# MIT-SPARK/Hydra-GNN

Hardware: AMD Instinct MI355X
Metric: scene-graphs/sec (fwd+bwd) MP3D hetero batch (higher is better)
Workload: dtype f32

## Files before the change

### hydra-gnn_amd/csrc/gemm.hip

```cpp
#include <algorithm>

#include "gemm_tile.h"

namespace hmp {

KT_DEFINE(gemm)

template <int ROWS, int BK>
using TileSide = TileSlots<256, ROWS, BK>;
template <int ROWS, int BK>
using TileRegs = StageRegs<TileSide<ROWS, BK>::NV>;

template <int ROWS, int BK>
__device__ __forceinline__ void tile_load_edge(TileRegs<ROWS, BK>& t, const float* __restrict__ p, int ld, int kcontig, int r0,
                                               int R, int n_real, int aug, int k0, int kend, int vec) {
  using S = TileSide<ROWS, BK>;
#pragma unroll
  for (int i = 0; i < S::NV; ++i) {
    float4 val = make_float4(0.f, 0.f, 0.f, 0.f);
    if (kcontig) {
      int r, k4;
      S::slot_rk(i, r, k4);
      const int gr = r0 + r, gk = k0 + k4;
      if (gr < R && gk < kend) {
// ... 405 lines not shown
    P.M = g.M; P.N = g.N; P.K = g.K; P.lda = g.lda; P.ldb = g.ldb; P.ldc = g.ldc; P.n_real = g.n_real; P.aug_ones = g.aug_ones;
    P.nslices = cdiv(g.N, TT_NS);
    int ks = (int)(512.0 * ((double)g.K * P.nslices / work_total) / P.nslices + 0.5);
    if (ks > GEMM_TALL_SLABS) ks = GEMM_TALL_SLABS;
    if (ks < 1) ks = 1;
    P.kchunk = g.kchunk = cdiv(cdiv(g.K, ks), TT_BK) * TT_BK;
    P.ksplit = g.ksplit = cdiv(g.K, P.kchunk);
    P.block_start = start;
    start += P.ksplit * P.nslices;
  }
  static const int rc = [] {
    return hipFuncSetAttribute(reinterpret_cast<const void*>(&gemm_tn_tall_kernel), hipFuncAttributeMaxDynamicSharedMemorySize,
                               2 * TT_STAGE * (int)sizeof(float)) == hipSuccess ? 0 : 1;
  }();
  HMP_CHECK_ARG(rc == 0, "gemm: could not raise the dynamic LDS limit of the tall weight-gradient kernel");
  hipLaunchKernelGGL(gemm_tn_tall_kernel, dim3(start), dim3(256), 2 * TT_STAGE * sizeof(float), st, tb);
  HMP_LAUNCH_CHECK();
  return HMP_OK;
}

int gemm_launch(GemmBatch& gb, bool want_split, int max_slabs, hipStream_t st) {
  HMP_CHECK_ARG(gb.n >= 0 && gb.n <= GEMM_MAX_PROB, "gemm: %d problems", gb.n);
  if (gemm_x3_takes(gb, want_split)) return gemm_x3_launch(gb, want_split, max_slabs, st);
  if (want_split) {
    GemmPeel tall;
    gemm_peel(gb, tall_takes, tall);
    if (tall.n_taken > 0) {
      HMP_TRY(tall_launch(gb, tall, st));
      return gemm_launch_rest(gb, tall, [&](GemmBatch& rest) { return gemm_launch(rest, want_split, max_slabs, st); });
    }
  }
  int64_t tiles64 = 0;
  double work = 0.0;
  int max_k = 0;
  for (int i = 0; i < gb.n; ++i) {
    const GemmProblem& p = gb.p[i];
    HMP_CHECK_ARG(p.M >= 0 && p.N >= 0 && p.K >= 0, "gemm: negative size");
    tiles64 += (int64_t)cdiv(p.M, 64) * cdiv(p.N, 64);
    work += (double)p.M * p.N * p.K;
    max_k = p.K > max_k ? p.K : max_k;
  }
  if (tiles64 >= 1024 || work >= 1e9) {
    int64_t tiles128 = 0;
    for (int i = 0; i < gb.n; ++i) tiles128 += (int64_t)cdiv(gb.p[i].M, 128) * cdiv(gb.p[i].N, 128);
    const bool big_ok = env_switch("HMP_GEMM_BIG") != '0';
    int min_n = 1 << 30;
    for (int i = 0; i < gb.n; ++i) min_n = gb.p[i].N < min_n ? gb.p[i].N : min_n;
    if (big_ok && min_n >= 256 && work >= 1e9 && (tiles128 >= 256 || (want_split && max_k >= 8192)))
      return launch_cfg<2, 2, 32, 2, 2>(gb, want_split, max_slabs, st);
    return launch_cfg<2, 2, 32>(gb, want_split, max_slabs, st);
  }
  if (max_k <= 64) return launch_cfg<1, 1, 64>(gb, want_split, max_slabs, st);
  return launch_cfg<1, 1, 128>(gb, want_split, max_slabs, st);
}

}

extern "C" int hmp_gemm_f32(const float* d_a, int32_t lda, int32_t trans_a, const float* d_b, int32_t ldb, int32_t trans_b,
                            float* d_c, int32_t ldc, int32_t M, int32_t N, int32_t K, void* stream) {
  using namespace hmp;
  HMP_CHECK_ARG(d_a && d_b && d_c, "hmp_gemm_f32: null pointer");
  HMP_CHECK_ARG(M >= 0 && N >= 0 && K >= 0, "hmp_gemm_f32: negative size");
  HMP_CHECK_ARG(lda >= (trans_a ? M : K) && ldb >= (trans_b ? K : N) && ldc >= N, "hmp_gemm_f32: leading dimension too small");
  GemmBatch gb;
  memset(&gb, 0, sizeof(gb));
  gb.n = 1;
  GemmProblem& p = gb.p[0];
  p.A = d_a; p.B = d_b; p.C = d_c;
  p.M = M; p.N = N; p.K = K;
  p.lda = lda; p.ldb = ldb; p.ldc = ldc;
  p.trans_a = trans_a; p.trans_b = trans_b;
  p.n_real = N;
  p.epi = EPI_NONE;
  if (M == 0 || N == 0) return HMP_OK;
  return gemm_launch(gb, false, 1, (hipStream_t)stream);
}

extern "C" int hmp_gemm_grouped(const hmp_gemm_desc* d, int32_t n, int32_t route, int32_t want_split, int32_t max_slabs,
                                int32_t* ksplit_out, void* stream) {
  using namespace hmp;
  static const bool have_device = hmp_device_count() > 0;
  HMP_CHECK_ARG(have_device, "hmp_gemm_grouped: no gfx950 device visible");
  HMP_CHECK_ARG((d || n == 0) && n >= 0 && n <= GEMM_MAX_PROB, "hmp_gemm_grouped: %d problems (at most %d)", n, GEMM_MAX_PROB);
  HMP_CHECK_ARG(route >= 0 && route <= 2 && max_slabs >= 1, "hmp_gemm_grouped: route %d, max_slabs %d", route, max_slabs);
  for (int i = 0; i < n; ++i) {
    const hmp_gemm_desc& q = d[i];
    HMP_CHECK_ARG(q.A && q.B && q.C, "hmp_gemm_grouped: null pointer (problem %d)", i);
    HMP_CHECK_ARG(q.M >= 0 && q.N >= 0 && q.K >= 0, "hmp_gemm_grouped: negative size (problem %d)", i);
    HMP_CHECK_ARG(q.n_real == q.N - (q.aug_ones ? 1 : 0) && q.n_real >= 0, "hmp_gemm_grouped: n_real %d, N %d, aug_ones %d (problem %d)",
                  q.n_real, q.N, q.aug_ones, i);
    HMP_CHECK_ARG(q.lda >= (q.trans_a ? q.M : q.K) && q.ldb >= (q.trans_b ? q.K : q.n_real) && q.ldc >= q.N,
                  "hmp_gemm_grouped: leading dimension too small (problem %d)", i);
    HMP_CHECK_ARG(q.epi == EPI_NONE || (q.epi == EPI_ACTMASK && q.H && q.ldh >= q.N), "hmp_gemm_grouped: epilogue (problem %d)", i);
    HMP_CHECK_ARG(!q.Cadd || q.ldadd >= q.N, "hmp_gemm_grouped: ldadd too small (problem %d)", i);
    HMP_CHECK_ARG(q.drop_p >= 0.f && q.drop_p < 1.f, "hmp_gemm_grouped: drop_p %g (problem %d)", (double)q.drop_p, i);
    HMP_CHECK_ARG(!want_split || q.M == 0 || q.slab_stride >= (int64_t)q.M * q.ldc, "hmp_gemm_grouped: slab_stride (problem %d)", i);
    HMP_CHECK_ARG(route == 1 || !(q.a_bf16 || q.b_bf16 || q.c_bf16 || q.h_bf16), "hmp_gemm_grouped: bf16 operands on route %d", route);
    HMP_CHECK_ARG(route != 2 || (q.trans_a && !q.trans_b && q.epi == EPI_NONE && !q.Cadd),
                  "hmp_gemm_grouped: the direct kernel takes the plain TN form only (problem %d)", i);
  }
  hipStream_t st = (hipStream_t)stream;
  if (route == 2) {
    TnBatch tb;
    memset(&tb, 0, sizeof(tb));
    tb.n = n;
    for (int i = 0; i < n; ++i) {
      const hmp_gemm_desc& q = d[i];
      TnProblem& P = tb.p[i];
      P.A = (const float*)q.A; P.B = (const float*)q.B; P.C = (float*)q.C; P.slab_stride = q.slab_stride;
      P.M = q.M; P.N = q.N; P.K = q.K; P.lda = q.lda; P.ldb = q.ldb; P.ldc = q.ldc;
      P.n_real = q.n_real; P.aug_ones = q.aug_ones;
    }
    int ok = 0;
    HMP_TRY(gemm_tn_direct_launch(tb, max_slabs, &ok, st));
    if (ksplit_out)
      for (int i = 0; i < n; ++i) ksplit_out[i] = ok ? tb.p[i].ksplit : 0;
    return HMP_OK;
  }
  GemmBatch gb;
  memset(&gb, 0, sizeof(gb));
  gb.n = n;
  for (int i = 0; i < n; ++i) {
    const hmp_gemm_desc& q = d[i];
    GemmProblem& p = gb.p[i];
    p.A = (const float*)q.A; p.B = (const float*)q.B; p.C = (float*)q.C; p.H = (const float*)q.H;
    p.a_bf16 = q.a_bf16; p.b_bf16 = q.b_bf16; p.c_bf16 = q.c_bf16; p.h_bf16 = q.h_bf16;
    p.slab_stride = q.slab_stride;
    p.M = q.M; p.N = q.N; p.K = q.K;
    p.lda = q.lda; p.ldb = q.ldb; p.ldc = q.ldc; p.ldh = q.ldh;
    p.trans_a = q.trans_a; p.trans_b = q.trans_b;
    p.n_real = q.n_real; p.aug_ones = q.aug_ones;
    p.epi = q.epi; p.act = q.act;
    p.drop_on = q.drop_p > 0.f ? 1 : 0;
    p.drop.thresh = drop_thresh(q.drop_p); p.drop.scale = 1.f / (1.f - q.drop_p);
    p.Cadd = q.Cadd; p.ldadd = q.ldadd;
  }
  const int rc = route == 0 ? gemm_launch(gb, want_split != 0, max_slabs, st) : gemm_bf16_launch(gb, want_split != 0, max_slabs, st);
  if (ksplit_out)
    for (int i = 0; i < n; ++i) ksplit_out[i] = gb.p[i].ksplit;
  return rc;
}
```

### hydra-gnn_amd/csrc/gemm_direct.hip

```cpp
#include "device_fns.h"

namespace hmp {

KT_DEFINE(gemmd)

typedef float f32x16 __attribute__((ext_vector_type(16)));

__device__ __forceinline__ void reduce4(f32x16& acc, float* red , int w, int lane, float (&out)[4]) {
#pragma unroll
  for (int i = 0; i < 16; ++i) red[(w * 16 + i) * 64 + lane] = acc[i];
  __syncthreads();
#pragma unroll
  for (int j = 0; j < 4; ++j) {
    const int i = 4 * w + j;
    out[j] = (red[(0 * 16 + i) * 64 + lane] + red[(1 * 16 + i) * 64 + lane]) + (red[(2 * 16 + i) * 64 + lane] + red[(3 * 16 + i) * 64 + lane]);
  }
}

constexpr int TN_MAXI = 24;

__global__ __launch_bounds__(256, 2) void gemm_tn_direct_kernel(const TnBatch tb) {
  __shared__ float red[4 * 16 * 64];
  const int blk = blockIdx.x;
  KT(8);
  karg_warm<(sizeof(TnBatch) + 63) / 64>(0, (int)sizeof(TnBatch));
  int pi = 0;
  while (pi + 1 < tb.n && blk >= tb.p[pi + 1].tile_start) ++pi;
  const TnProblem& P = tb.p[pi];
  const int local = blk - P.tile_start;
  const int z = local % P.ksplit, t = local / P.ksplit;
  const int tm = t / P.tiles_n, tn = t % P.tiles_n;
  const int m0 = tm * 32, n0 = tn * 32;
  const int lane = threadIdx.x & 63, w = threadIdx.x >> 6;
  const int r = lane & 31, h = lane >> 5;
  const int kbeg = z * P.kchunk, kend = min(P.K, kbeg + P.kchunk);
  const int n_steps = (kend - kbeg + 1) >> 1;
  const int per = (n_steps + 3) >> 2;
  const int s0 = w * per, s1 = min(n_steps, s0 + per);
  const int am = min(m0 + r, P.M - 1);
  const int bn = n0 + r;
  const bool b_real = bn < P.n_real;
  const bool b_one = P.aug_ones && bn == P.n_real;
  const int bnc = b_real ? bn : 0;
  f32x16 acc;
#pragma unroll
  for (int i = 0; i < 16; ++i) acc[i] = 0.f;
  for (int sb0 = s0; sb0 < s1; sb0 += TN_MAXI) {
    float av[TN_MAXI], bv[TN_MAXI];
#pragma unroll
    for (int i = 0; i < TN_MAXI; ++i) {
      const int k = kbeg + 2 * (sb0 + i) + h;
      const bool live = (sb0 + i < s1) && k < kend;
      const int kc = live ? k : kbeg;
      const float a = P.A[(int64_t)kc * P.lda + am];
      const float b = P.B[(int64_t)kc * P.ldb + bnc];
      av[i] = live ? a : 0.f;
      bv[i] = live ? (b_real ? b : (b_one ? 1.f : 0.f)) : 0.f;
    }
#pragma unroll
    for (int i = 0; i < TN_MAXI; ++i)
      if (sb0 + i < s1) acc = __builtin_amdgcn_mfma_f32_32x32x2f32(av[i], bv[i], acc, 0, 0, 0);
  }
  float out[4];
  reduce4(acc, red, w, lane, out);
  float* C = P.C + (int64_t)z * P.slab_stride;
  const int col = n0 + (lane & 31);
  if (col < P.N) {
#pragma unroll
    for (int j = 0; j < 4; ++j) {
      const int row = m0 + j + 8 * w + 4 * h;
      if (row < P.M) C[(int64_t)row * P.ldc + col] = out[j];
    }
  }
  KT(9);
}

int gemm_tn_direct_launch(TnBatch& tb, int max_slabs, int* ok, hipStream_t st) {
  int start = 0;
  *ok = 1;
  for (int i = 0; i < tb.n; ++i) {
    TnProblem& P = tb.p[i];
    P.tiles_m = cdiv(P.M, 32);
    P.tiles_n = cdiv(P.N, 32);
    const int trips = (P.tiles_m * P.tiles_n >= 512) ? 4 : 2;
    int ks = cdiv(P.K, 2 * 4 * TN_MAXI * trips);
    if (ks < 1) ks = 1;
    if (ks > max_slabs) { *ok = 0; return HMP_OK; }
    while (ks * 2 <= max_slabs && cdiv(P.K, ks * 2) >= 32 && P.tiles_m * P.tiles_n * ks < 256) ks *= 2;
    int kchunk = cdiv(cdiv(P.K, ks), 2) * 2;
    if (kchunk < 2) kchunk = 2;
    ks = P.K > 0 ? cdiv(P.K, kchunk) : 1;
    P.ksplit = ks;
    P.kchunk = kchunk;
    P.tile_start = start;
    start += P.tiles_m * P.tiles_n * ks;
  }
  tb.total_tiles = start;
  if (start == 0) return HMP_OK;
  hipLaunchKernelGGL(gemm_tn_direct_kernel, dim3(start), dim3(256), 0, st, tb);
  HMP_LAUNCH_CHECK();
  return HMP_OK;
}

}
```

### hydra-gnn_amd/csrc/kernels.h

```cpp
#pragma once
#include "common.h"

namespace hmp {

enum { EPI_NONE = 0, EPI_ACTMASK = 1 };

struct GemmProblem {
  const float* A;
  const float* B;
  float* C;
  const float* H;
  int c_bf16;
  int a_bf16;
  int b_bf16;
  int h_bf16;
  const float* A2;
  int lda2, a_split;
  int64_t slab_stride;
  int M, N, K;
  int lda, ldb, ldc, ldh;
  int trans_a;
  int trans_b;
  int n_real;
  int aug_ones;
// ... 83 lines not shown
    gb.p[s.rest_idx[i]].kchunk = s.rest.p[i].kchunk;
  }
  return rc;
}

struct XcdGrid {
  int groups, tiles_per_group;
};
inline XcdGrid xcd_set_grid(int per_cu, int n_slices, int n_tiles) {
  int sets = per_cu * device_cu_count() / (8 * n_slices);
  if (sets < 1) sets = 1;
  int groups = 8 * sets;
  if (groups > n_tiles) groups = ((n_tiles + 7) / 8) * 8;
  return {groups, cdiv(n_tiles, groups)};
}

int gemm_launch(GemmBatch& gb, bool want_split, int max_slabs, hipStream_t st);
int gemm_bf16_launch(GemmBatch& gb, bool want_split, int max_slabs, hipStream_t st);
bool gemm_x3_takes(const GemmBatch& gb, bool want_split);
bool gemm_x3_split_takes(const GemmProblem* ps, int n);
int gemm_x3_launch(GemmBatch& gb, bool want_split, int max_slabs, hipStream_t st);
bool gemm_bf16_dx_takes(const GemmProblem& p, bool want_split);
int gemm_bf16_dx_launch(const GemmProblem& p, hipStream_t st);
bool gemm_bf16_dw_takes(const GemmProblem& p, bool want_split);
int gemm_bf16_dw_launch(const GemmProblem& p, int max_slabs, int* n_slabs, hipStream_t st);

constexpr int FR_MAX_PROB = 4;
constexpr int FR_MAX_SEG = 6;
constexpr int FR_MAX_SRC = 6;
struct FrontSeg {
  int col0, rows, nsrc, ld;
  uint32_t off[FR_MAX_SRC];
};
struct FrontProb {
  const float* A;
  float* C;
  int lda, ldc, M, N, K;
  int n_seg, max_nsrc, vec;
  int blk_start, tiles_m, tiles_n;
  FrontSeg seg[FR_MAX_SEG];
};
struct FrontJob {
  const int64_t* ei;
  int E, n_src, n_dst;
  uint32_t rowptr, col, eid, t_rowptr, t_col, t_eid, tmp_in, tmp_out, pos_of_eid, degf, flags;
  const int64_t *gp_dst, *gp_src, *gp_edge;
  int n_graphs;
};
struct PackSeg;
struct NetState;
struct FrontArgs {
  int gemm_blocks, plan_blocks, pack_blocks;
  int n_prob, n_jobs, need_tpos, plan_rc;
  const float* params;
  char* ws;
  int* status;
  const PackSeg* segs;
  const int2* pack_map;
  float* packed;
  int* step_ctr;
  int* step_mirror;
  int prob_start[FR_MAX_PROB];
  int part_start[2 * HMP_MAX_EDGE_TYPES + 1];
  int rows_per_part[2 * HMP_MAX_EDGE_TYPES];
  FrontJob job[HMP_MAX_EDGE_TYPES];
  FrontProb prob[FR_MAX_PROB];
};
int front_launch(FrontArgs& a, hipStream_t st);

struct TnProblem {
  const float* A;
  const float* B;
  float* C;
  int64_t slab_stride;
  int M, N, K, lda, ldb, ldc;
  int n_real, aug_ones;
  int ksplit, kchunk, tile_start, tiles_m, tiles_n;
};
struct TnBatch {
  int n, total_tiles;
  TnProblem p[GEMM_MAX_PROB];
};
int gemm_tn_direct_launch(TnBatch& tb, int max_slabs, int* ok, hipStream_t st);

struct PlanJob {
  const int64_t* ei;
  int64_t E;
  int n_src, n_dst;
  int *rowptr, *col, *eid, *t_rowptr, *t_col, *t_pos;
  float* degf;
  const int64_t *gp_dst, *gp_src, *gp_edge;
  int n_graphs;
  int *cnt_in, *cnt_out, *cur_in, *cur_out;
  int* flags;
  int *tmp_in, *tmp_out, *t_eid, *pos_of_eid;
  int *tmpc_in, *tmpc_out;
};
struct PlanBatch {
  int n;
  int need_tpos;
  int clear_first;
  int build_id;
  int* flags_all;
  int64_t edge_start[HMP_MAX_EDGE_TYPES + 1];
  int64_t row_start[2 * HMP_MAX_EDGE_TYPES + 1];
  PlanJob j[HMP_MAX_EDGE_TYPES];
};
__host__ __device__ inline bool plan_edge_ok(int64_t s, int64_t d, int n_src, int n_dst) {
  return s >= 0 && s < n_src && d >= 0 && d < n_dst;
}
size_t plan_scratch_ints(int64_t E, int n_src, int n_dst);
void plan_carve(PlanJob& job, int* scratch);
int plan_launch(PlanBatch& pb, int* d_status, hipStream_t st);
int plan_link_launch(PlanBatch& pb, hipStream_t st);

constexpr int AGG_MAX_IN = 6;
struct AggIn {
  const int* rowptr;
  const int* col;
  const float* z;
  int ldz, coff;
  int same_type;
  int n_src;
};
struct AggDst {
  int n_rows, F;
  float* out;
  int ldo;
  const float* zroot;
  int ldzr, roff;
  const float* bias;
  int n_in;
  int act;
  int drop_on;
  DropCfg drop;
  int block_start;
  const float* pw;
  float* pz;
  int pldw, pldz, pncols, pK;
  const int64_t* ce_labels;
  int64_t ce_ignored;
  int ce_classes, ce_ldg;
  float* ce_grad;
  float* ce_row_lv;
  const uint8_t* ce_mask;
  const float* ce_weight;
  int ce_tail;
  int win_in;
  int tile_rows;
  AggIn in[AGG_MAX_IN];
};
struct AggArgs {
  int n;
  int total_blocks;
  int mean;
  int xcd;
  int zb16;
  int hb16;
  NetState* state;
  int bstart[HMP_MAX_NODE_TYPES];
  AggDst d[HMP_MAX_NODE_TYPES];
};
int agg_fwd_launch(AggArgs& a, hipStream_t st);
int agg_proj_fwd_launch(AggArgs& a, hipStream_t st);

struct TAggOut {
// ... 310 lines not shown
```

### hydra-gnn_amd/csrc/net.hip

```cpp
#include <cstdlib>
#include <vector>

#include "plan_small.h"

using namespace hmp;

namespace {

struct ConvLayout {
  int coff;
  int asoff, adoff;
  int H, C, Cp;
  int64_t vedge_off;
  int64_t vslab_off;
  bool wd_is_src;
  float *smax, *sden, *alpha_drop, *dlogit, *dlogit_orig;
  bool agg_first;
  int aoff, ld_m;
  int64_t wc_off, cslab_off;
  float *mrows, *dmrows;
};

struct LayerLayout {
  int kind;
  int n_live;
  int live[HMP_MAX_CONVS];
  ConvLayout conv[HMP_MAX_CONVS];
  int n_in[HMP_MAX_NODE_TYPES];
  bool reads[HMP_MAX_NODE_TYPES];
  int aggf_of_src[HMP_MAX_NODE_TYPES];
  int ncols[HMP_MAX_NODE_TYPES];
  int roff[HMP_MAX_NODE_TYPES];
  int64_t wp_off[HMP_MAX_NODE_TYPES];
  int ldw[HMP_MAX_NODE_TYPES];
  int64_t wpt_off[HMP_MAX_NODE_TYPES];
  int ldt[HMP_MAX_NODE_TYPES];
  int64_t bias_off[HMP_MAX_NODE_TYPES];
  int64_t slab_off[HMP_MAX_NODE_TYPES];
  int lddw[HMP_MAX_NODE_TYPES];
  int64_t bslab_off[HMP_MAX_NODE_TYPES];
  GatLayerS* d_gat;
  GatLayerS h_gat;
};

constexpr int MAX_SLABS = 192;
static_assert(MAX_SLABS >= GEMM_TALL_SLABS, "the slab buffer must hold what the tall weight-gradient kernel may write");
constexpr int TN_DIRECT_SLABS = 16;

struct ProfRec {
  int cls;
  hipEvent_t a, b;
};

}

struct EnvSwitches {
  bool plan_sliced = true;
  bool front = true;
  bool z16 = true;
  bool h16 = true;
  bool rootcopy = false;
  bool tn_direct = true;
  bool bf16_all = false;
};

struct StepCall {
  int training = 0;
  uint64_t seed = 0;
  uint32_t rng_step = 0;
  int* d_step = nullptr;
  const int64_t* ce_labels = nullptr;
  const hmp_head_targets* tgt = nullptr;
  int64_t ce_ignored = 0;
  AdamFuse adam = {};
  bool fin_loss = false;
  int fin_rows = 0;
  bool aux_g_ready = false;
  int head_blocks = 0;
  bool ce_done = false;
  bool tail_done[2] = {false, false};
  bool adam_done = false;
};

struct hmp_net {
  hmp_net_spec spec;
  EnvSwitches env;
  int T, ET, L;
  int dim[HMP_MAX_LAYERS + 1][HMP_MAX_NODE_TYPES];
  int ld[HMP_MAX_LAYERS + 1][HMP_MAX_NODE_TYPES];
  LayerLayout lay[HMP_MAX_LAYERS];
  int64_t packed_floats, slab_floats;
  int out_dim, out_ld;
  bool any_gat = false;
  bool pass0[HMP_MAX_NODE_TYPES] = {false};

  PackSeg* d_pack_segs = nullptr;
  int n_pack = 0;
  int64_t pack_rows = 0;
  GradSeg* d_grad_segs = nullptr;
  int n_grad = 0;
  int64_t grad_elems = 0;
  int max_pack_rows = 0;
  int64_t max_grad_elems = 0;
  SegBlocks pack_sb, grad_sb;
  int2* d_pack_map = nullptr;
  int n_pack_blocks16 = 0;
  char* ws_base = nullptr;
  size_t ws_bytes = 0;
  float* degf[HMP_MAX_EDGE_TYPES];
  bool any_agg_first = false;
  int* d_iota = nullptr;
  float* d_ones = nullptr;
  float* d_sadd = nullptr;
  int iota_cap = 0;
  int64_t sadd_floats = 0;
  float* d_row_lv = nullptr;

  bool bound = false;
  int cap_nodes[HMP_MAX_NODE_TYPES];
  int64_t cap_edges[HMP_MAX_EDGE_TYPES];
  NetState* d_state = nullptr;
  hmp_plan plan[HMP_MAX_EDGE_TYPES];
  int* plan_scratch[HMP_MAX_EDGE_TYPES];
  float* d_packed = nullptr;
  float* d_slabs = nullptr;
  float* H[HMP_MAX_LAYERS + 1][HMP_MAX_NODE_TYPES];
  float* G[HMP_MAX_LAYERS + 1][HMP_MAX_NODE_TYPES];
  bool h16[HMP_MAX_LAYERS + 1][HMP_MAX_NODE_TYPES] = {};
  float* Z[HMP_MAX_LAYERS][HMP_MAX_NODE_TYPES];
  float* dZ[HMP_MAX_LAYERS][HMP_MAX_NODE_TYPES];
  float* d_out = nullptr;
  float* d_gout = nullptr;
  int cap_out = 0;

  bool have_fwd = false;
  bool plan_ok = false;
  hmp_batch batch;
  int training = 0;
  uint64_t seed = 0;
  uint32_t rng_step = 0;
  GradReduceDyn dyn;
  StepCall call;

  int compute_bf16 = 0;
  int fuse_mode = -1;
  bool fuse_now = false;
  bool reuse_plan = false;
  bool has_heads = false;
  hmp_linear_heads heads = {};
  int64_t head_slab_off = 0, head_slab_stride = 0;
  int head_ld_slab = 0;
  bool has_pools = false;
  int head_pool[2] = {-1, -1};
  float* d_dpool[2] = {nullptr, nullptr};
  const float* class_w[2] = {nullptr, nullptr};

  bool prof = false;
  std::vector<ProfRec> recs;
};

namespace {

void read_env(hmp_net* n) {
  EnvSwitches e;
  e.plan_sliced = env_switch("HMP_PLAN_SLICED") != '0';
  e.front = env_switch("HMP_FRONT") != '0';
  e.z16 = env_switch("HMP_Z16") != '0';
  e.h16 = env_switch("HMP_H16") != '0';
  e.rootcopy = env_switch("HMP_ROOTCOPY") == '1';
  e.tn_direct = env_switch("HMP_TN") != '0';
  e.bf16_all = env_switch("HMP_BF16_ALL") == '1';
  n->env = e;
}

inline int fpad(int f) { return align4(f); }

inline int head_type(const hmp_net* n, int h) { return h == 0 ? n->spec.readout_type : n->spec.aux_readout_type; }
inline int label_type(const hmp_net* n, int h) {
  return n->head_pool[h] >= 0 ? n->spec.edge_dst[n->head_pool[h]] : head_type(n, h);
}

int build_layout(hmp_net* n) {
  const hmp_net_spec& S = n->spec;
  n->T = S.n_node_types; n->ET = S.n_edge_types; n->L = S.n_layers;
  HMP_CHECK_ARG(n->T >= 1 && n->T <= HMP_MAX_NODE_TYPES, "net: n_node_types %d", n->T);
  HMP_CHECK_ARG(n->ET >= 1 && n->ET <= HMP_MAX_EDGE_TYPES, "net: n_edge_types %d", n->ET);
  HMP_CHECK_ARG(n->L >= 1 && n->L <= HMP_MAX_LAYERS, "net: n_layers %d", n->L);
  HMP_CHECK_ARG(S.readout_type >= 0 && S.readout_type < n->T, "net: readout_type");
  HMP_CHECK_ARG(S.pool_edge_type >= -1 && S.pool_edge_type < n->ET, "net: pool_edge_type");
  HMP_CHECK_ARG(S.aux_readout_type >= -1 && S.aux_readout_type < n->T && S.aux_readout_type != S.readout_type &&
                    (S.aux_readout_type < 0 || S.pool_edge_type < 0),
                "net: aux_readout_type (a second node type, not with a pooled output)");
  for (int e = 0; e < n->ET; ++e)
    HMP_CHECK_ARG(S.edge_src[e] >= 0 && S.edge_src[e] < n->T && S.edge_dst[e] >= 0 && S.edge_dst[e] < n->T, "net: edge type %d endpoints", e);
  for (int t = 0; t < n->T; ++t) {
    n->dim[0][t] = S.in_dim[t];
    n->ld[0][t] = 0;
  }
  int64_t packed = 0, slabs = 0;
  for (int l = 0; l < n->L; ++l) {
    const hmp_layer_spec& Ls = S.layers[l];
    LayerLayout& Y = n->lay[l];
    HMP_CHECK_ARG(Ls.n_convs >= 1 && Ls.n_convs <= HMP_MAX_CONVS, "net: layer %d has %d convs", l, Ls.n_convs);
    Y.kind = Ls.convs[0].kind;
    Y.d_gat = nullptr;
    HMP_CHECK_ARG(Y.kind == HMP_CONV_SAGE || Y.kind == HMP_CONV_GAT, "net: layer %d: unknown conv kind %d", l, Y.kind);
    HMP_CHECK_ARG(Ls.group_mean == 0 || Y.kind == HMP_CONV_GAT, "net: HeteroConv aggr=mean is only supported for GAT layers");
    for (int t = 0; t < n->T; ++t) {
      n->dim[l + 1][t] = Ls.out_dim[t];
      n->ld[l + 1][t] = fpad(Ls.out_dim[t]);
      if (Ls.passthrough[t]) {
        HMP_CHECK_ARG(l == 0 && n->L > 1, "net: passthrough node types are supported on the first layer only");
        HMP_CHECK_ARG(Ls.out_dim[t] == S.in_dim[t], "net: passthrough type %d must keep its input width", t);
        n->pass0[t] = true;
      }
      Y.ncols[t] = 0;
      Y.roff[t] = -1;
      Y.n_in[t] = 0;
      Y.reads[t] = false;
      Y.aggf_of_src[t] = -1;
    }
    Y.n_live = 0;
    int n_outgoing[HMP_MAX_NODE_TYPES] = {0};
    for (int c = 0; c < Ls.n_convs; ++c) {
      const hmp_conv_spec& C = Ls.convs[c];
      ConvLayout& Q = Y.conv[c];
      memset(&Q, 0, sizeof(Q));
      HMP_CHECK_ARG(C.kind == Y.kind, "net: layer %d mixes conv kinds", l);
      HMP_CHECK_ARG(C.edge_type >= 0 && C.edge_type < n->ET, "net: conv edge_type");
      HMP_CHECK_ARG(C.src == S.edge_src[C.edge_type] && C.dst == S.edge_dst[C.edge_type], "net: conv endpoints disagree with edge type");
      HMP_CHECK_ARG(n->dim[l][C.src] > 0 && n->dim[l][C.dst] > 0, "net: layer %d conv %d reads a node type with no features", l, c);
      if (Y.kind == HMP_CONV_SAGE) {
        HMP_CHECK_ARG(C.f_out == Ls.out_dim[C.dst], "net: SAGE f_out must equal the layer's out_dim of the destination type");
      } else {
        HMP_CHECK_ARG(gat_shape_ok(C.heads, C.f_out), "net: GAT heads %d / channels %d unsupported (at most %d channels per head, at most %d heads above 256 channels)",
                      C.heads, C.f_out, GAT_CMAX, GAT_WIDE_HMAX);
        HMP_CHECK_ARG(Ls.out_dim[C.dst] == (C.concat ? C.heads * C.f_out : C.f_out), "net: GAT out_dim mismatch on layer %d conv %d", l, c);
        HMP_CHECK_ARG(C.edge_dim >= 0 && C.edge_dim <= GAT_MAX_EDIM, "net: GAT edge_dim %d > %d", C.edge_dim, GAT_MAX_EDIM);
        HMP_CHECK_ARG(!(C.edge_dim > 0 && C.fill_mean && C.self_loops), "net: fill_value='mean' with edge attributes is not supported (the reference passes zeros)");
        HMP_CHECK_ARG(!C.self_loops || C.src == C.dst, "net: self loops need src == dst (the reference sets add_self_loops = (src == dst))");
      }
      HMP_CHECK_ARG(!C.agg_first || (Y.kind == HMP_CONV_SAGE && C.src != C.dst), "net: agg_first is for SAGE convs between two node types");
      if (!C.active) continue;
      Y.live[Y.n_live++] = c;
      ++Y.n_in[C.dst];
      const bool aggf = C.agg_first != 0;
      ++n_outgoing[aggf ? C.dst : C.src];
      HMP_CHECK_ARG(Y.n_in[C.dst] <= AGG_MAX_IN && n_outgoing[C.src] <= AGG_MAX_IN && n_outgoing[C.dst] <= AGG_MAX_IN,
                    "net: more than %d convs share a node type", AGG_MAX_IN);
      Y.reads[C.src] = Y.reads[C.dst] = true;
      if (Y.kind == HMP_CONV_SAGE) {
        HMP_CHECK_ARG(C.w0 >= 0 && C.b0 >= 0 && C.w1 >= 0, "net: SAGE conv needs lin_l.weight, lin_l.bias, lin_r.weight");
        if (aggf) {
// ... 1205 lines not shown
        if (Y.ncols[s] == 0 || b->n_nodes[s] == 0) continue;
        GemmProblem p;
        memset(&p, 0, sizeof(p));
        p.A = n->dZ[l][s]; p.lda = Y.ncols[s]; p.trans_a = 1;
        p.a_bf16 = dz16 ? 1 : 0;
        if (rootless && Y.roff[s] >= 0) { int ldg; p.A2 = g_of(s, ldg); p.lda2 = ldg; p.a_split = Y.roff[s]; }
        p.B = h_ptr(n, l, s); p.ldb = h_ld(n, l, s); p.trans_b = 0;
        p.b_bf16 = n->h16[l][s] ? 1 : 0;
        p.C = n->d_slabs + Y.slab_off[s]; p.ldc = Y.lddw[s];
        p.slab_stride = (int64_t)Y.ncols[s] * Y.lddw[s];
        p.M = Y.ncols[s]; p.N = n->dim[l][s] + 1; p.K = b->n_nodes[s];
        p.n_real = n->dim[l][s]; p.aug_ones = 1;
        add(slab_id_w(l, s), p);
      }
      for (int i = 0; i < Y.n_live; ++i) {
        const int c = Y.live[i];
        if (!aggf_live(c)) continue;
        const hmp_conv_spec& C = Ls.convs[c];
        const ConvLayout& Q = Y.conv[c];
        GemmProblem p;
        memset(&p, 0, sizeof(p));
        p.A = dz_at(C.dst, Q.aoff); p.lda = Y.ncols[C.dst]; p.trans_a = 1; p.a_bf16 = dz16 ? 1 : 0;
        p.B = Q.mrows; p.ldb = Q.ld_m; p.trans_b = 0;
        p.C = n->d_slabs + Q.cslab_off; p.ldc = Y.lddw[C.src];
        p.slab_stride = (int64_t)fpad(C.f_out) * Y.lddw[C.src];
        p.M = fpad(C.f_out); p.N = n->dim[l][C.src]; p.K = b->n_nodes[C.dst];
        p.n_real = p.N; p.aug_ones = 0;
        add(slab_id_v(l, c), p);
      }
      if (Y.kind == HMP_CONV_GAT) {
        for (int t = 0; t < n->T; ++t) {
          if (Y.n_in[t] == 0 || b->n_nodes[t] == 0) continue;
          int ldg;
          const float* g = g_of(t, ldg);
          GemmProblem p;
          memset(&p, 0, sizeof(p));
          p.A = g; p.lda = ldg; p.trans_a = 1;
          p.B = g; p.ldb = ldg; p.trans_b = 0;
          p.C = n->d_slabs + Y.bslab_off[t]; p.ldc = 4;
          p.slab_stride = (int64_t)fpad(Ls.out_dim[t]) * 4;
          p.M = Ls.out_dim[t]; p.N = 1; p.K = b->n_nodes[t];
          p.n_real = 0; p.aug_ones = 1;
          add(slab_id_b(l, t), p);
        }
        for (int i = 0; i < Y.n_live; ++i) {
          const int c = Y.live[i];
          const hmp_conv_spec& C = Ls.convs[c];
          if (C.edge_dim == 0 || b->n_edges[C.edge_type] == 0) continue;
          GemmProblem p;
          memset(&p, 0, sizeof(p));
          p.A = b->d_edge_attr[C.edge_type]; p.lda = C.edge_dim; p.trans_a = 1;
          p.B = Y.conv[c].dlogit_orig; p.ldb = GAT_HMAX; p.trans_b = 0;
          p.C = n->d_slabs + Y.conv[c].vslab_off; p.ldc = GAT_HMAX;
          p.slab_stride = GAT_MAX_EDIM * GAT_HMAX;
          p.M = C.edge_dim; p.N = C.heads; p.K = (int)b->n_edges[C.edge_type];
          p.n_real = C.heads;
          add(slab_id_v(l, c), p);
        }
      }
    }
  }
  if (skip_w) return HMP_OK;
  {
    Scope sc(n, KC_GEMM_BWD, st);
    std::vector<int> ks;
    bool direct = n->fuse_now;
    if (direct) {
      if (!n->env.tn_direct) direct = false;
      if (direct && !n->compute_bf16 && !wps.empty() && gemm_x3_split_takes(wps.data(), (int)wps.size())) direct = false;
      for (size_t i = 0; i < wps.size() && direct; ++i)
        if (wps[i].K > TN_DIRECT_SLABS * 384 || wps[i].b_bf16 || wps[i].a_bf16) direct = false;
      for (size_t base = 0; base < wps.size() && direct; base += GEMM_MAX_PROB) {
        TnBatch tb;
        memset(&tb, 0, sizeof(tb));
        const size_t cnt = (wps.size() - base) < (size_t)GEMM_MAX_PROB ? (wps.size() - base) : (size_t)GEMM_MAX_PROB;
        for (size_t i = 0; i < cnt; ++i) {
          const GemmProblem& g = wps[base + i];
          TnProblem& P = tb.p[tb.n++];
          P.A = g.A; P.B = g.B; P.C = g.C; P.slab_stride = g.slab_stride;
          P.M = g.M; P.N = g.N; P.K = g.K; P.lda = g.lda; P.ldb = g.ldb; P.ldc = g.ldc;
          P.n_real = g.n_real; P.aug_ones = g.aug_ones;
        }
        int ok = 0;
        HMP_TRY(gemm_tn_direct_launch(tb, TN_DIRECT_SLABS, &ok, st));
        HMP_CHECK_ARG(ok, "net: weight-gradient problem too deep for the direct kernel after the size check");
        for (size_t i = 0; i < cnt; ++i) ks.push_back(tb.p[i].ksplit);
      }
    }
    if (!direct) HMP_TRY(gemm_many(n, wps, true, st, &ks));
    for (size_t i = 0; i < wids.size(); ++i) n->dyn.n_slabs[wids[i]] = (unsigned char)ks[i];
  }
  {
    Scope sc(n, KC_GRAD_REDUCE, st);
    const int64_t na = n->spec.n_active_params;
    AdamFuse af = n->call.adam;
    af.on = (af.on && fin_early && !n->any_gat) ? 1 : 0;
    n->call.adam_done = af.on != 0;
    HMP_TRY(grad_reduce_launch(n->d_grad_segs, n->grad_sb, n->dyn, n->d_slabs, d_params, d_grads,
                               n->call.fin_loss ? n->d_row_lv : nullptr, n->call.fin_rows > 0 ? n->call.fin_rows : b->n_out, d_grads + na, n->d_state,
                               af, st));
    n->call.fin_loss = false;
  }
  return HMP_OK;
}

struct StepGuard {
  hmp_net* n;
  StepGuard(hmp_net* net, int training = 0, uint64_t seed = 0, uint32_t rng_step = 0, int* d_step = nullptr) : n(net) {
    read_env(n);
    n->call.training = training; n->call.seed = seed; n->call.rng_step = rng_step;
    n->call.d_step = d_step;
  }
  ~StepGuard() { n->call = StepCall(); }
  StepGuard(const StepGuard&) = delete;
  StepGuard& operator=(const StepGuard&) = delete;
};

int plain_forward(hmp_net* n, const hmp_batch* b, const float* d_params, hipStream_t st, int training = 0, uint64_t seed = 0,
                  uint32_t rng_step = 0) {
  StepGuard guard(n, training, seed, rng_step);
  return forward_impl(n, b, d_params, st);
}

}

extern "C" int hmp_net_create(const hmp_net_spec* spec, hmp_net** out) {
  HMP_CHECK_ARG(spec && out, "hmp_net_create: null argument");
  HMP_CHECK_ARG(hmp_device_count() > 0, "hmp_net_create: no gfx950 device visible");
  hmp_net* n = new hmp_net;
  n->spec = *spec;
  int r = build_layout(n);
  if (r == HMP_OK) r = build_tables(n);
  if (r == HMP_OK) {
    if (hipMalloc(&n->d_state, 256) != hipSuccess || hipMemset(n->d_state, 0, 256) != hipSuccess) {
      snprintf(err_buf(), 512, "hmp_net_create: device allocation of the net state failed");
      r = HMP_E_HIP;
    }
  }
  if (r == HMP_OK) {
    const int fz = env_switch("HMP_FUSE");
    n->fuse_mode = fz < 0 ? -1 : fz == '1' ? 1 : 0;
  }
  if (r != HMP_OK) {
    hmp_net_destroy(n);
    return r;
  }
  *out = n;
  return HMP_OK;
}

extern "C" void hmp_net_destroy(hmp_net* n) {
  if (!n) return;
  for (auto& r : n->recs) { (void)hipEventDestroy(r.a); (void)hipEventDestroy(r.b); }
  if (n->d_state) (void)hipFree(n->d_state);
  if (n->d_pack_segs) (void)hipFree(n->d_pack_segs);
  if (n->d_pack_map) (void)hipFree(n->d_pack_map);
  if (n->d_grad_segs) (void)hipFree(n->d_grad_segs);
  for (int l = 0; l < HMP_MAX_LAYERS; ++l)
    if (l < n->L && n->lay[l].d_gat) (void)hipFree(n->lay[l].d_gat);
  delete n;
}

extern "C" size_t hmp_net_workspace_bytes(const hmp_net* net, const int32_t* cap_nodes, const int64_t* cap_edges) {
  if (!net || !cap_nodes || !cap_edges) return 0;
  hmp_net tmp = *net;
  tmp.recs.clear();
  return carve(&tmp, nullptr, cap_nodes, cap_edges);
// ... 730 lines not shown
```

Baseline: 375,400.

## Add single-round TN weight-gradient kernel with VALU bias-column sums

Adds a variant of the direct TN weight-gradient GEMM that sizes K-chunks so the whole grid fits in one wave of resident blocks (3 per CU), loads all A/B values up front in groups, and sorts problems by chunk length. When the augmented ones column sits on a 32-column boundary, it computes that bias-gradient column as a plain sum of A on the VALU instead of spending a whole MFMA tile on it. Net code tries this launch first under a new env switch and falls back to the old kernel if the grid would exceed one round. The larger per-thread register arrays and higher blocks-per-CU bound may raise register pressure or cause spills.

```diff
diff --git a/hydra-gnn_amd/csrc/gemm.hip b/hydra-gnn_amd/csrc/gemm.hip
--- a/hydra-gnn_amd/csrc/gemm.hip
+++ b/hydra-gnn_amd/csrc/gemm.hip
@@ -511,7 +511,7 @@
   static const bool have_device = hmp_device_count() > 0;
   HMP_CHECK_ARG(have_device, "hmp_gemm_grouped: no gfx950 device visible");
   HMP_CHECK_ARG((d || n == 0) && n >= 0 && n <= GEMM_MAX_PROB, "hmp_gemm_grouped: %d problems (at most %d)", n, GEMM_MAX_PROB);
-  HMP_CHECK_ARG(route >= 0 && route <= 2 && max_slabs >= 1, "hmp_gemm_grouped: route %d, max_slabs %d", route, max_slabs);
+  HMP_CHECK_ARG(route >= 0 && route <= 3 && max_slabs >= 1, "hmp_gemm_grouped: route %d, max_slabs %d", route, max_slabs);
   for (int i = 0; i < n; ++i) {
     const hmp_gemm_desc& q = d[i];
     HMP_CHECK_ARG(q.A && q.B && q.C, "hmp_gemm_grouped: null pointer (problem %d)", i);
@@ -525,11 +525,11 @@
     HMP_CHECK_ARG(q.drop_p >= 0.f && q.drop_p < 1.f, "hmp_gemm_grouped: drop_p %g (problem %d)", (double)q.drop_p, i);
     HMP_CHECK_ARG(!want_split || q.M == 0 || q.slab_stride >= (int64_t)q.M * q.ldc, "hmp_gemm_grouped: slab_stride (problem %d)", i);
     HMP_CHECK_ARG(route == 1 || !(q.a_bf16 || q.b_bf16 || q.c_bf16 || q.h_bf16), "hmp_gemm_grouped: bf16 operands on route %d", route);
-    HMP_CHECK_ARG(route != 2 || (q.trans_a && !q.trans_b && q.epi == EPI_NONE && !q.Cadd),
+    HMP_CHECK_ARG(route < 2 || (q.trans_a && !q.trans_b && q.epi == EPI_NONE && !q.Cadd),
                   "hmp_gemm_grouped: the direct kernel takes the plain TN form only (problem %d)", i);
   }
   hipStream_t st = (hipStream_t)stream;
-  if (route == 2) {
+  if (route >= 2) {
     TnBatch tb;
     memset(&tb, 0, sizeof(tb));
     tb.n = n;
@@ -541,7 +541,7 @@
       P.n_real = q.n_real; P.aug_ones = q.aug_ones;
     }
     int ok = 0;
-    HMP_TRY(gemm_tn_direct_launch(tb, max_slabs, &ok, st));
+    HMP_TRY(route == 2 ? gemm_tn_direct_launch(tb, max_slabs, &ok, st) : gemm_tn_round_launch(tb, max_slabs, &ok, st));
     if (ksplit_out)
       for (int i = 0; i < n; ++i) ksplit_out[i] = ok ? tb.p[i].ksplit : 0;
     return HMP_OK;
diff --git a/hydra-gnn_amd/csrc/gemm_direct.hip b/hydra-gnn_amd/csrc/gemm_direct.hip
--- a/hydra-gnn_amd/csrc/gemm_direct.hip
+++ b/hydra-gnn_amd/csrc/gemm_direct.hip
@@ -3,6 +3,7 @@
 namespace hmp {
 
 KT_DEFINE(gemmd)
+KT_BLOCKS_DEFINE(gemmd)
 
 typedef float f32x16 __attribute__((ext_vector_type(16)));
 
@@ -18,11 +19,46 @@
 }
 
 constexpr int TN_MAXI = 24;
-
-__global__ __launch_bounds__(256, 2) void gemm_tn_direct_kernel(const TnBatch tb) {
-  __shared__ float red[4 * 16 * 64];
+constexpr int TN_ROUND_MAXI = 48;
+constexpr int TN_ROUND_BPC = 3;
+constexpr int TN_ROUND_GROUP = 8;
+
+template <int MAXI, bool HAS_B>
+__device__ __forceinline__ void tn_round_trip(const float* __restrict__ A, const float* __restrict__ B, int lda, int ldb, int am, int bnc,
+                                              bool b_real, float b_fill, int kbeg, int k0, int kend, int cnt, f32x16& acc, float& asum) {
+  float av[MAXI], bv[MAXI];
+#pragma unroll
+  for (int g = 0; g < MAXI; g += TN_ROUND_GROUP) {
+    if (g < cnt) {
+#pragma unroll
+      for (int i = g; i < g + TN_ROUND_GROUP; ++i) {
+        const int k = k0 + 2 * i;
+        const int kc = (i < cnt && k < kend) ? k : kbeg;
+        av[i] = A[(int64_t)kc * lda + am];
+        if constexpr (HAS_B) bv[i] = B[(int64_t)kc * ldb + bnc];
+      }
+    }
+  }
+#pragma unroll
+  for (int g = 0; g < MAXI; g += TN_ROUND_GROUP) {
+    if (g < cnt) {
+#pragma unroll
+      for (int i = g; i < g + TN_ROUND_GROUP; ++i) {
+        const bool live = i < cnt && k0 + 2 * i < kend;
+        const float a = live ? av[i] : 0.f;
+        asum += a;
+        if constexpr (HAS_B) acc = __builtin_amdgcn_mfma_f32_32x32x2f32(a, live ? (b_real ? bv[i] : b_fill) : 0.f, acc, 0, 0, 0);
+      }
+    }
+  }
+}
+
+template <int MAXI, int BPC, bool ROUND>
+__global__ __launch_bounds__(256, BPC) void gemm_tn_direct_kernel(const TnBatch tb) {
+  __shared__ float red[4 * 16 * 64 + (ROUND ? 4 * 32 : 0)];
   const int blk = blockIdx.x;
   KT(8);
+  KT_BLOCK_BEGIN();
   karg_warm<(sizeof(TnBatch) + 63) / 64>(0, (int)sizeof(TnBatch));
   int pi = 0;
   while (pi + 1 < tb.n && blk >= tb.p[pi + 1].tile_start) ++pi;
@@ -39,40 +75,63 @@
   const int s0 = w * per, s1 = min(n_steps, s0 + per);
   const int am = min(m0 + r, P.M - 1);
   const int bn = n0 + r;
+  const bool ones_valu = ROUND && P.aug_ones && (P.n_real & 31) == 0;
+  const int n_mfma = ones_valu ? P.n_real : P.N;
   const bool b_real = bn < P.n_real;
-  const bool b_one = P.aug_ones && bn == P.n_real;
+  const bool b_one = P.aug_ones && bn == P.n_real && !ones_valu;
   const int bnc = b_real ? bn : 0;
   f32x16 acc;
 #pragma unroll
   for (int i = 0; i < 16; ++i) acc[i] = 0.f;
-  for (int sb0 = s0; sb0 < s1; sb0 += TN_MAXI) {
-    float av[TN_MAXI], bv[TN_MAXI];
-#pragma unroll
-    for (int i = 0; i < TN_MAXI; ++i) {
-      const int k = kbeg + 2 * (sb0 + i) + h;
-      const bool live = (sb0 + i < s1) && k < kend;
-      const int kc = live ? k : kbeg;
-      const float a = P.A[(int64_t)kc * P.lda + am];
-      const float b = P.B[(int64_t)kc * P.ldb + bnc];
-      av[i] = live ? a : 0.f;
-      bv[i] = live ? (b_real ? b : (b_one ? 1.f : 0.f)) : 0.f;
-    }
-#pragma unroll
-    for (int i = 0; i < TN_MAXI; ++i)
-      if (sb0 + i < s1) acc = __builtin_amdgcn_mfma_f32_32x32x2f32(av[i], bv[i], acc, 0, 0, 0);
-  }
-  float out[4];
-  reduce4(acc, red, w, lane, out);
+  bool has_b = true;
+  bool sum_a = false;
+  if constexpr (ROUND) {
+    has_b = n0 < P.n_real;
+    sum_a = ones_valu && tn == 0;
+    const int cnt = __builtin_amdgcn_readfirstlane(s1 - s0);
+    float asum = 0.f;
+    if (has_b) tn_round_trip<MAXI, true>(P.A, P.B, P.lda, P.ldb, am, bnc, b_real, b_one ? 1.f : 0.f, kbeg, kbeg + 2 * s0 + h, kend, cnt, acc, asum);
+    else tn_round_trip<MAXI, false>(P.A, P.B, P.lda, P.ldb, am, bnc, b_real, 0.f, kbeg, kbeg + 2 * s0 + h, kend, cnt, acc, asum);
+    if (sum_a) {
+      asum += __shfl_xor(asum, 32);
+      if (h == 0) red[4 * 16 * 64 + w * 32 + r] = asum;
+    }
+  } else {
+    for (int sb0 = s0; sb0 < s1; sb0 += MAXI) {
+      float av[MAXI], bv[MAXI];
+#pragma unroll
+      for (int i = 0; i < MAXI; ++i) {
+        const int k = kbeg + 2 * (sb0 + i) + h;
+        const bool live = (sb0 + i < s1) && k < kend;
+        const int kc = live ? k : kbeg;
+        const float a = P.A[(int64_t)kc * P.lda + am];
+        const float b = P.B[(int64_t)kc * P.ldb + bnc];
+        av[i] = live ? a : 0.f;
+        bv[i] = live ? (b_real ? b : (b_one ? 1.f : 0.f)) : 0.f;
+      }
+#pragma unroll
+      for (int i = 0; i < MAXI; ++i)
+        if (sb0 + i < s1) acc = __builtin_amdgcn_mfma_f32_32x32x2f32(av[i], bv[i], acc, 0, 0, 0);
+    }
+  }
+  float out[4] = {0.f, 0.f, 0.f, 0.f};
+  if (has_b) reduce4(acc, red, w, lane, out);
+  else __syncthreads();
   float* C = P.C + (int64_t)z * P.slab_stride;
   const int col = n0 + (lane & 31);
-  if (col < P.N) {
+  if (has_b && col < n_mfma) {
 #pragma unroll
     for (int j = 0; j < 4; ++j) {
       const int row = m0 + j + 8 * w + 4 * h;
       if (row < P.M) C[(int64_t)row * P.ldc + col] = out[j];
     }
   }
+  if (sum_a && w == 0 && h == 0 && m0 + r < P.M) {
+    const float* s = red + 4 * 16 * 64 + r;
+    C[(int64_t)(m0 + r) * P.ldc + P.n_real] = (s[0] + s[32]) + (s[64] + s[96]);
+  }
   KT(9);
+  KT_BLOCK_END();
 }
 
 int gemm_tn_direct_launch(TnBatch& tb, int max_slabs, int* ok, hipStream_t st) {
@@ -97,9 +156,51 @@
   }
   tb.total_tiles = start;
   if (start == 0) return HMP_OK;
-  hipLaunchKernelGGL(gemm_tn_direct_kernel, dim3(start), dim3(256), 0, st, tb);
+  hipLaunchKernelGGL((gemm_tn_direct_kernel<TN_MAXI, 2, false>), dim3(start), dim3(256), 0, st, tb);
   HMP_LAUNCH_CHECK();
   return HMP_OK;
 }
 
-}
+int gemm_tn_round_launch(TnBatch& tb, int max_slabs, int* ok, hipStream_t st) {
+  constexpr int cap = 2 * 4 * TN_ROUND_MAXI;
+  const int64_t slots = (int64_t)TN_ROUND_BPC * device_cu_count();
+  *ok = 0;
+  TnBatch lb;
+  memset(&lb, 0, sizeof(lb));
+  int64_t total = 0;
+  for (int i = 0; i < tb.n; ++i) {
+    TnProblem P = tb.p[i];
+    const bool ones_valu = P.aug_ones && (P.n_real & 31) == 0;
+    P.tiles_m = cdiv(P.M, 32);
+    P.tiles_n = P.N <= 0 ? 0 : (ones_valu ? (P.n_real >= 32 ? P.n_real / 32 : 1) : cdiv(P.N, 32));
+    int ks = cdiv(P.K, cap);
+    if (ks < 1) ks = 1;
+    if (ks > max_slabs) return HMP_OK;
+    int kchunk = cdiv(cdiv(P.K, ks), 2) * 2;
+    if (kchunk < 2) kchunk = 2;
+    P.kchunk = kchunk;
+    P.ksplit = P.K > 0 ? cdiv(P.K, kchunk) : 1;
+    total += (int64_t)P.tiles_m * P.tiles_n * P.ksplit;
+    if (total > slots) return HMP_OK;
+    int at = lb.n++;
+    while (at > 0 && lb.p[at - 1].kchunk < kchunk) { lb.p[at] = lb.p[at - 1]; --at; }
+    lb.p[at] = P;
+    lb.p[at].tile_start = i;
+  }
+  *ok = 1;
+  int start = 0;
+  for (int j = 0; j < lb.n; ++j) {
+    TnProblem& P = lb.p[j];
+    const int i = P.tile_start;
+    P.tile_start = start;
+    start += P.tiles_m * P.tiles_n * P.ksplit;
+    tb.p[i] = P;
+  }
+  lb.total_tiles = tb.total_tiles = start;
+  if (start == 0) return HMP_OK;
+  hipLaunchKernelGGL((gemm_tn_direct_kernel<TN_ROUND_MAXI, TN_ROUND_BPC, true>), dim3(start), dim3(256), 0, st, lb);
+  HMP_LAUNCH_CHECK();
+  return HMP_OK;
+}
+
+}
diff --git a/hydra-gnn_amd/csrc/kernels.h b/hydra-gnn_amd/csrc/kernels.h
--- a/hydra-gnn_amd/csrc/kernels.h
+++ b/hydra-gnn_amd/csrc/kernels.h
@@ -189,6 +189,7 @@
   TnProblem p[GEMM_MAX_PROB];
 };
 int gemm_tn_direct_launch(TnBatch& tb, int max_slabs, int* ok, hipStream_t st);
+int gemm_tn_round_launch(TnBatch& tb, int max_slabs, int* ok, hipStream_t st);
 
 struct PlanJob {
   const int64_t* ei;
diff --git a/hydra-gnn_amd/csrc/net.hip b/hydra-gnn_amd/csrc/net.hip
--- a/hydra-gnn_amd/csrc/net.hip
+++ b/hydra-gnn_amd/csrc/net.hip
@@ -61,6 +61,7 @@
   bool h16 = true;
   bool rootcopy = false;
   bool tn_direct = true;
+  bool dw_round = true;
   bool bf16_all = false;
 };
 
@@ -169,6 +170,7 @@
   e.h16 = env_switch("HMP_H16") != '0';
   e.rootcopy = env_switch("HMP_ROOTCOPY") == '1';
   e.tn_direct = env_switch("HMP_TN") != '0';
+  e.dw_round = env_switch("HMP_DW_ROUND") != '0';
   e.bf16_all = env_switch("HMP_BF16_ALL") == '1';
   n->env = e;
 }
@@ -1540,7 +1542,8 @@
           P.n_real = g.n_real; P.aug_ones = g.aug_ones;
         }
         int ok = 0;
-        HMP_TRY(gemm_tn_direct_launch(tb, TN_DIRECT_SLABS, &ok, st));
+        if (n->env.dw_round) HMP_TRY(gemm_tn_round_launch(tb, TN_DIRECT_SLABS, &ok, st));
+        if (!ok) HMP_TRY(gemm_tn_direct_launch(tb, TN_DIRECT_SLABS, &ok, st));
         HMP_CHECK_ARG(ok, "net: weight-gradient problem too deep for the direct kernel after the size check");
         for (size_t i = 0; i < cnt; ++i) ks.push_back(tb.p[i].ksplit);
       }
```

Result: slower. 371,600 (-1.0%).
